# facebookresearch/sylph-few-shot-detection

Measured on AMD Instinct MI355X. Metric: query images/sec, R50-FPN 5-way 5-shot 800x1333 (whole job), higher is better.
Workload: dtype bf16

## Files before the change

### sylph-few-shot-detection_amd/csrc/stem_conv.hip

```cpp
#include "gfx950.h"
#include "kernels.h"

namespace sylph {

namespace {
constexpr int PP = 48;
constexpr int PROWS = 21, PCOLS = 38;
constexpr int PATCH_BYTES = 8192;
constexpr int SCP = 68;
constexpr int NLOAD = (PROWS * PCOLS + 255) / 256;
}

__global__ __launch_bounds__(256, 2) void stem_conv_kernel(const bf16_t* __restrict__ x, const bf16_t* __restrict__ wp,
                                                           const float* __restrict__ scale, const float* __restrict__ shift,
                                                           bf16_t* __restrict__ out, int H, int W, int H2, int W2,
                                                           int tiles_y, int tiles_x, int ntiles) {
  extern __shared__ __attribute__((aligned(16))) char smem[];
  char* patch = smem;
  float* sC = reinterpret_cast<float*>(smem + PATCH_BYTES);
  const int tid = threadIdx.x, lane = tid & 63, wave = tid >> 6, l31 = lane & 31, lh = lane >> 5;

  bf16x8 wb[14][2];
#pragma unroll
  for (int ks = 0; ks < 14; ++ks)
#pragma unroll
    for (int j = 0; j < 2; ++j) wb[ks][j] = *reinterpret_cast<const bf16x8*>(wp + (j * 32 + l31) * 224 + ks * 16 + lh * 8);

  const int m = wave * 32 + l31, py = m >> 4, px = m & 15;
  const int aoff = ((2 * py) * PP + 2 * px + 2 * lh) * 8;

  const int c8 = tid & 7, rr = tid >> 3;
  float sc[8], sh[8];
#pragma unroll
  for (int h = 0; h < 2; ++h) {
    const float4 s4 = reinterpret_cast<const float4*>(scale + c8 * 8)[h], b4 = reinterpret_cast<const float4*>(shift + c8 * 8)[h];
    sc[4 * h] = s4.x; sc[4 * h + 1] = s4.y; sc[4 * h + 2] = s4.z; sc[4 * h + 3] = s4.w;
    sh[4 * h] = b4.x; sh[4 * h + 1] = b4.y; sh[4 * h + 2] = b4.z; sh[4 * h + 3] = b4.w;
  }

  int f_pr[NLOAD], f_pc[NLOAD], f_lds[NLOAD];
  uint32_t f_in = 0;
#pragma unroll
  for (int r = 0; r < NLOAD; ++r) {
    const int idx = tid + 256 * r;
    f_pr[r] = idx / PCOLS; f_pc[r] = idx - f_pr[r] * PCOLS;
    f_lds[r] = (f_pr[r] * PP + f_pc[r]) * 8;
    f_in |= (idx < PROWS * PCOLS ? 1u : 0u) << r;
  }

  auto fetch = [&](int tile_in, uint2 (&v)[NLOAD], uint32_t& okmask) {
    const int tile = tile_in < ntiles ? tile_in : ntiles - 1;
    const int tx = tile % tiles_x, t2 = tile / tiles_x, ty = t2 % tiles_y, b = t2 / tiles_y;
    const int iy0 = ty * 16 - 3, ix0 = tx * 32 - 3;
    okmask = 0;
    const bf16_t* xb = x + (size_t)b * H * W * 4;
#pragma unroll
    for (int r = 0; r < NLOAD; ++r) {
      const int iy = iy0 + f_pr[r], ix = ix0 + f_pc[r];
      const bool ok = ((f_in >> r) & 1u) && (unsigned)iy < (unsigned)H && (unsigned)ix < (unsigned)W;
      const int cy = min(max(iy, 0), H - 1), cx = min(max(ix, 0), W - 1);
      const bf16_t* src = xb + (cy * W + cx) * 4;
      asm volatile("global_load_dwordx2 %0, %1, off" : "=v"(v[r]) : "v"(src) : "memory");
      okmask |= (ok ? 1u : 0u) << r;
    }
  };
  auto park = [&](const uint2 (&v)[NLOAD], uint32_t okmask) {
#pragma unroll
    for (int r = 0; r < NLOAD; ++r) {
      const uint2 t = ((okmask >> r) & 1u) ? v[r] : make_uint2(0u, 0u);
      if ((f_in >> r) & 1u) *reinterpret_cast<uint2*>(patch + f_lds[r]) = t;
    }
  };

#pragma unroll
  for (int ks = 0; ks < 14; ++ks)
#pragma unroll
    for (int j = 0; j < 2; ++j) asm volatile("" : "+v"(wb[ks][j]));
#pragma unroll
  for (int e = 0; e < 8; ++e) { asm volatile("" : "+v"(sc[e])); asm volatile("" : "+v"(sh[e])); }

  const int g = gridDim.x;
  auto do_tile = [&](int tile, uint2 (&q)[NLOAD], uint32_t& qm) {
    wait_vmcnt<4>();
    static_assert(NLOAD == 4, "the vmcnt immediate above is NLOAD");
    park(q, qm);
    lds_barrier();
    fetch(tile + 2 * g, q, qm);

    f32x16 acc[2];
#pragma unroll
    for (int j = 0; j < 2; ++j)
#pragma unroll
      for (int r = 0; r < 16; ++r) acc[j][r] = 0.f;
#pragma unroll
    for (int kh = 0; kh < 7; ++kh)
#pragma unroll
      for (int h = 0; h < 2; ++h) {
        const bf16x8 fa = *reinterpret_cast<const bf16x8*>(patch + aoff + (kh * PP + 4 * h) * 8);
#pragma unroll
        for (int j = 0; j < 2; ++j) acc[j] = __builtin_amdgcn_mfma_f32_32x32x16_bf16(wb[kh * 2 + h][j], fa, acc[j], 0, 0, 0);
      }

    const int tx = tile % tiles_x, t2 = tile / tiles_x, ty = t2 % tiles_y, b = t2 / tiles_y;
    const int oy0 = ty * 8, ox0 = tx * 16;
#pragma unroll
    for (int p = 0; p < 2; ++p) {
      if (p > 0) lds_barrier();
      if ((wave >> 1) == p) {
#pragma unroll
        for (int j = 0; j < 2; ++j)
#pragma unroll
          for (int q4 = 0; q4 < 4; ++q4)
            *reinterpret_cast<float4*>(sC + ((wave & 1) * 32 + l31) * SCP + j * 32 + 8 * q4 + 4 * lh) =
                make_float4(acc[j][4 * q4], acc[j][4 * q4 + 1], acc[j][4 * q4 + 2], acc[j][4 * q4 + 3]);
      }
      lds_barrier();
#pragma unroll
      for (int it = 0; it < 2; ++it) {
        const int rl = rr + 32 * it, mm = p * 64 + rl;
        const int oy = oy0 + (mm >> 4), ox = ox0 + (mm & 15);
        if (oy < H2 && ox < W2) {
          const float4 lo = *reinterpret_cast<const float4*>(sC + rl * SCP + c8 * 8);
          const float4 hi = *reinterpret_cast<const float4*>(sC + rl * SCP + c8 * 8 + 4);
          float v[8] = {lo.x, lo.y, lo.z, lo.w, hi.x, hi.y, hi.z, hi.w};
#pragma unroll
          for (int e = 0; e < 8; ++e) { v[e] = v[e] * sc[e] + sh[e]; v[e] = v[e] > 0.f ? v[e] : 0.f; }
          store8<bf16_t>(out + (((size_t)b * H2 + oy) * W2 + ox) * 64 + c8 * 8, v);
        }
      }
    }
    lds_barrier();
  };

  uint2 qa[NLOAD], qb[NLOAD];
  uint32_t ma, mb;
  int tile = blockIdx.x;
  fetch(tile, qa, ma);
  fetch(tile + g, qb, mb);
  while (tile < ntiles) {
    do_tile(tile, qa, ma);
    tile += g;
    if (tile >= ntiles) break;
    do_tile(tile, qb, mb);
    tile += g;
  }
}

namespace {
constexpr int FR = 17, FC = 15;
constexpr int FPR = 8, FPC = 7;
constexpr int FPROWS = 2 * FR + 5, FPCOLS = 36;
constexpr int FPATCH_BYTES = 15104;
constexpr int FTP = 144;
constexpr int FTILE_BYTES = FR * FC * FTP;
constexpr int FNLOAD = (FPROWS * FPCOLS + 255) / 256;
constexpr int FLDS = FPATCH_BYTES + ((FTILE_BYTES + 127) / 128) * 128 + 128 * 4;
}

struct StemRawArgs { const ImageDesc* imgs; int B; float m0, m1, m2, is0, is1, is2; };

template <bool RAW>
__global__ __launch_bounds__(256, 2) void stem_pool_kernel(const bf16_t* __restrict__ x, const StemRawArgs raw, const bf16_t* __restrict__ wp,
                                                           const float* __restrict__ scale, const float* __restrict__ shift,
                                                           bf16_t* __restrict__ out, char* __restrict__ trash, int H, int W, int H2,
                                                           int W2, int H4, int W4, int tiles_y, int tiles_x, int ntiles) {
  constexpr int NV = RAW ? 3 * FNLOAD : FNLOAD;
  extern __shared__ __attribute__((aligned(16))) char smem[];
  char* patch = smem;
  char* st = smem + FPATCH_BYTES;
  float* ss = reinterpret_cast<float*>(smem + FPATCH_BYTES + ((FTILE_BYTES + 127) / 128) * 128);
  ImageDesc* descs = reinterpret_cast<ImageDesc*>(smem + FLDS);
  const int tid = threadIdx.x, lane = tid & 63, wave = tid >> 6, l31 = lane & 31, lh = lane >> 5;
  if (RAW)
    for (int i = tid; i < raw.B; i += 256) descs[i] = raw.imgs[i];

  bf16x8 wb[14][2];
#pragma unroll
  for (int ks = 0; ks < 14; ++ks)
#pragma unroll
    for (int j = 0; j < 2; ++j) wb[ks][j] = *reinterpret_cast<const bf16x8*>(wp + (j * 32 + l31) * 224 + ks * 16 + lh * 8);
  if (tid < 128) ss[tid] = tid < 64 ? scale[tid] : shift[tid - 64];

  int aoff[2], sy[2], sx[2], toff[2];
#pragma unroll
  for (int p = 0; p < 2; ++p) {
    const int m = min(p * 128 + wave * 32 + l31, FR * FC - 1);
    sy[p] = m / FC;
    sx[p] = m - sy[p] * FC;
    aoff[p] = ((2 * sy[p]) * PP + 2 * sx[p] + 2 * lh) * 8;
    toff[p] = (p * 128 + wave * 32 + l31 < FR * FC) ? m * FTP + 8 * lh : -1;
  }
  int f_pr[FNLOAD], f_pc[FNLOAD], f_lds[FNLOAD];
  uint32_t f_in = 0;
#pragma unroll
  for (int r = 0; r < FNLOAD; ++r) {
    const int idx = tid + 256 * r;
    f_pr[r] = idx / FPCOLS; f_pc[r] = idx - f_pr[r] * FPCOLS;
    f_lds[r] = (f_pr[r] * PP + f_pc[r]) * 8;
    f_in |= (idx < FPROWS * FPCOLS ? 1u : 0u) << r;
  }
  int p_off[2], p_oy[2], p_ox[2];
#pragma unroll
  for (int r = 0; r < 2; ++r) {
    const int idx = tid + 256 * r, pp = idx >> 3;
    p_oy[r] = pp / FPC; p_ox[r] = pp - p_oy[r] * FPC;
    p_off[r] = pp < FPR * FPC ? ((2 * p_oy[r]) * FC + 2 * p_ox[r]) * FTP + (idx & 7) * 16 : -1;
  }
  char* const my_trash = trash + ((size_t)blockIdx.x * 256 + tid) * 16;

  auto tile_origin = [&](int tile, int& b, int& oy0, int& ox0) {
    const int tx = tile % tiles_x, t2 = tile / tiles_x, ty = t2 % tiles_y;
    b = t2 / tiles_y; oy0 = ty * FPR; ox0 = tx * FPC;
  };
  auto fetch = [&](int tile_in, unsigned (&v)[3 * FNLOAD], uint32_t& okmask) {
    int b, oy0, ox0;
    tile_origin(tile_in < ntiles ? tile_in : ntiles - 1, b, oy0, ox0);
    const int iy0 = 4 * oy0 - 5, ix0 = 4 * ox0 - 5;
    okmask = 0;
    if (RAW) {
      const ImageDesc d = descs[b];
      const size_t plane = (size_t)d.h * d.w;
#pragma unroll
      for (int r = 0; r < FNLOAD; ++r) {
        const int iy = iy0 + f_pr[r], ix = ix0 + f_pc[r];
        const bool ok = ((f_in >> r) & 1u) && (unsigned)iy < (unsigned)d.h && (unsigned)ix < (unsigned)d.w;
        const int cy = min(max(iy, 0), d.h - 1), cx = min(max(ix, 0), d.w - 1);
        const float* src = d.ptr + (size_t)cy * d.w + cx;
        asm volatile("global_load_dword %0, %1, off" : "=v"(v[3 * r]) : "v"(src) : "memory");
        asm volatile("global_load_dword %0, %1, off" : "=v"(v[3 * r + 1]) : "v"(src + plane) : "memory");
        asm volatile("global_load_dword %0, %1, off" : "=v"(v[3 * r + 2]) : "v"(src + 2 * plane) : "memory");
        okmask |= (ok ? 1u : 0u) << r;
      }
    } else {
      const bf16_t* xb = x + (size_t)b * H * W * 4;
#pragma unroll
      for (int r = 0; r < FNLOAD; ++r) {
        const int iy = iy0 + f_pr[r], ix = ix0 + f_pc[r];
        const bool ok = ((f_in >> r) & 1u) && (unsigned)iy < (unsigned)H && (unsigned)ix < (unsigned)W;
        const int cy = min(max(iy, 0), H - 1), cx = min(max(ix, 0), W - 1);
        const bf16_t* src = xb + (cy * W + cx) * 4;
        uint2 t;
        asm volatile("global_load_dwordx2 %0, %1, off" : "=v"(t) : "v"(src) : "memory");
        v[2 * r] = t.x; v[2 * r + 1] = t.y;
        okmask |= (ok ? 1u : 0u) << r;
      }
    }
  };
  auto park = [&](const unsigned (&v)[3 * FNLOAD], uint32_t okmask) {
#pragma unroll
    for (int r = 0; r < FNLOAD; ++r) {
      uint2 t = make_uint2(0u, 0u);
      if ((okmask >> r) & 1u) {
        if (RAW) {
          bf16x2 lo2;
          lo2[0] = (bf16_t)((__uint_as_float(v[3 * r]) - raw.m0) * raw.is0);
          lo2[1] = (bf16_t)((__uint_as_float(v[3 * r + 1]) - raw.m1) * raw.is1);
          bf16x2 hi2;
          hi2[0] = (bf16_t)((__uint_as_float(v[3 * r + 2]) - raw.m2) * raw.is2);
          hi2[1] = (bf16_t)0.f;
          t = make_uint2(__builtin_bit_cast(unsigned, lo2), __builtin_bit_cast(unsigned, hi2));
        } else {
          t = make_uint2(v[2 * r], v[2 * r + 1]);
        }
      }
      if ((f_in >> r) & 1u) *reinterpret_cast<uint2*>(patch + f_lds[r]) = t;
    }
  };
#pragma unroll
  for (int ks = 0; ks < 14; ++ks)
#pragma unroll
    for (int j = 0; j < 2; ++j) asm volatile("" : "+v"(wb[ks][j]));
  wait_vmcnt<0>();
  if (RAW) __syncthreads();

  const int g = gridDim.x;
  int nth = 0;
  auto do_tile = [&](int tile, unsigned (&q)[3 * FNLOAD], uint32_t& qm) {
    static_assert(FNLOAD == 6, "the vmcnt immediates below are NV = 6 / 18 (+ 2 stores per finished tile)");
    if (nth == 0) wait_vmcnt<NV>();
    else if (nth == 1) wait_vmcnt<NV + 2>();
    else wait_vmcnt<NV + 4>();
    ++nth;
    park(q, qm);
    lds_barrier();
    fetch(tile + 2 * g, q, qm);
    int b, oy0, ox0;
    tile_origin(tile, b, oy0, ox0);
    const int sy0 = 2 * oy0 - 1, sx0 = 2 * ox0 - 1;
#pragma unroll
    for (int p = 0; p < 2; ++p) {
      f32x16 acc[2];
#pragma unroll
      for (int j = 0; j < 2; ++j)
#pragma unroll
        for (int r = 0; r < 16; ++r) acc[j][r] = 0.f;
#pragma unroll
      for (int kh = 0; kh < 7; ++kh)
#pragma unroll
        for (int h = 0; h < 2; ++h) {
          const bf16x8 fa = *reinterpret_cast<const bf16x8*>(patch + aoff[p] + (kh * PP + 4 * h) * 8);
#pragma unroll
          for (int j = 0; j < 2; ++j) acc[j] = __builtin_amdgcn_mfma_f32_32x32x16_bf16(wb[kh * 2 + h][j], fa, acc[j], 0, 0, 0);
        }
      const bool inimg = (unsigned)(sy0 + sy[p]) < (unsigned)H2 && (unsigned)(sx0 + sx[p]) < (unsigned)W2;
      const unsigned keep = inimg ? 0xffffffffu : 0u;
      if (toff[p] >= 0) {
#pragma unroll
        for (int j = 0; j < 2; ++j)
#pragma unroll
          for (int q4 = 0; q4 < 4; ++q4) {
            const int n0 = 32 * j + 8 * q4 + 4 * lh;
            const f32x4 sv = *reinterpret_cast<const f32x4*>(ss + n0), bv = *reinterpret_cast<const f32x4*>(ss + 64 + n0);
            u32x2 o;
#pragma unroll
            for (int hh = 0; hh < 2; ++hh) {
              bf16x2 v2;
              v2[0] = (bf16_t)(acc[j][4 * q4 + 2 * hh] * sv[2 * hh] + bv[2 * hh]);
              v2[1] = (bf16_t)(acc[j][4 * q4 + 2 * hh + 1] * sv[2 * hh + 1] + bv[2 * hh + 1]);
              const s16x2 z = {0, 0};
              o[hh] = __builtin_bit_cast(unsigned, __builtin_elementwise_max(__builtin_bit_cast(s16x2, v2), z)) & keep;
            }
            *reinterpret_cast<u32x2*>(st + toff[p] + 64 * j + 16 * q4) = o;
          }
      }
    }
    lds_barrier();
#pragma unroll
    for (int r = 0; r < 2; ++r) {
      typedef unsigned short u16x8 __attribute__((ext_vector_type(8)));
      u16x8 mx = {0, 0, 0, 0, 0, 0, 0, 0};
      if (p_off[r] >= 0) {
#pragma unroll
        for (int dy = 0; dy < 3; ++dy)
#pragma unroll
          for (int dx = 0; dx < 3; ++dx)
            mx = __builtin_elementwise_max(mx, *reinterpret_cast<const u16x8*>(st + p_off[r] + (dy * FC + dx) * FTP));
      }
      const int oy = oy0 + p_oy[r], ox = ox0 + p_ox[r];
      const bool okp = p_off[r] >= 0 && oy < H4 && ox < W4;
      char* dst = okp ? reinterpret_cast<char*>(out) + ((((size_t)b * H4 + oy) * W4 + ox) * 64 + (tid & 7) * 8) * 2 : my_trash;
      *reinterpret_cast<u16x8*>(dst) = mx;
    }
    lds_barrier();
  };

  unsigned qa[3 * FNLOAD], qb[3 * FNLOAD];
  uint32_t ma, mb;
  int tile = blockIdx.x;
  fetch(tile, qa, ma);
  fetch(tile + g, qb, mb);
  while (tile < ntiles) {
    do_tile(tile, qa, ma);
    tile += g;
    if (tile >= ntiles) break;
    do_tile(tile, qb, mb);
    tile += g;
  }
}

int launch_stem_pool(const void* x, const void* wp, const float* scale, const float* shift, void* out, void* trash, int B, int H, int W,
                     int H2, int W2, int H4, int W4, hipStream_t s) {
  const int tiles_y = (H4 + FPR - 1) / FPR, tiles_x = (W4 + FPC - 1) / FPC, ntiles = B * tiles_y * tiles_x;
  const int grid = ntiles < 512 ? ntiles : 512;
  hipLaunchKernelGGL(stem_pool_kernel<false>, dim3(grid), dim3(256), FLDS, s, (const bf16_t*)x, StemRawArgs{}, (const bf16_t*)wp, scale, shift,
                     (bf16_t*)out, (char*)trash, H, W, H2, W2, H4, W4, tiles_y, tiles_x, ntiles);
  return (int)hipGetLastError();
}

int launch_stem_pool_raw(const ImageDesc* imgs_dev, const float* mean, const float* stdv, const void* wp, const float* scale,
                         const float* shift, void* out, void* trash, int B, int H, int W, int H2, int W2, int H4, int W4, hipStream_t s) {
  if (B > STEM_RAW_MAX_BATCH) return -1;
  const int tiles_y = (H4 + FPR - 1) / FPR, tiles_x = (W4 + FPC - 1) / FPC, ntiles = B * tiles_y * tiles_x;
  const int grid = ntiles < 512 ? ntiles : 512;
  const StemRawArgs raw{imgs_dev, B, mean[0], mean[1], mean[2], 1.f / stdv[0], 1.f / stdv[1], 1.f / stdv[2]};
  hipLaunchKernelGGL(stem_pool_kernel<true>, dim3(grid), dim3(256), FLDS + (size_t)B * sizeof(ImageDesc), s, (const bf16_t*)nullptr, raw,
                     (const bf16_t*)wp, scale, shift, (bf16_t*)out, (char*)trash, H, W, H2, W2, H4, W4, tiles_y, tiles_x, ntiles);
  return (int)hipGetLastError();
}

int launch_stem_conv(const void* x, const void* wp, const float* scale, const float* shift, void* out, int B, int H, int W, int H2,
                     int W2, hipStream_t s) {
  const int tiles_y = (H2 + 7) / 8, tiles_x = (W2 + 15) / 16, ntiles = B * tiles_y * tiles_x;
  const int grid = ntiles < 512 ? ntiles : 512;
  const size_t lds = PATCH_BYTES + (size_t)64 * SCP * 4;
  hipLaunchKernelGGL(stem_conv_kernel, dim3(grid), dim3(256), lds, s, (const bf16_t*)x, (const bf16_t*)wp, scale, shift, (bf16_t*)out,
                     H, W, H2, W2, tiles_y, tiles_x, ntiles);
  return (int)hipGetLastError();
}

}
```

Before: 2334.

## Software-pipeline LDS reads and interleave next-tile fetches with MFMA in stem pool kernel

Reworks the fused stem conv+maxpool kernel. The double-buffered two-tiles-ahead prefetch becomes a single buffer whose global loads for the next tile are issued one chunk at a time between MFMA steps. LDS reads for the A fragments, the scale/shift values and the pooling taps are issued ahead through inline-asm ds_read_b128 with explicit lgkmcnt waits, so LDS latency overlaps compute. The patch layout gets padding (FPP 46 plus extra bytes every two rows) and the pooling lanes are remapped, presumably to reduce bank conflicts. In exchange the prefetch distance drops to one tile, which may expose more global-load latency, and the hand-written waitcnt counts are fragile.

After: 2331. Within noise of the previous version (-0.1%).

```diff
diff --git a/sylph-few-shot-detection_amd/csrc/stem_conv.hip b/sylph-few-shot-detection_amd/csrc/stem_conv.hip
--- a/sylph-few-shot-detection_amd/csrc/stem_conv.hip
+++ b/sylph-few-shot-detection_amd/csrc/stem_conv.hip
@@ -1,3 +1,5 @@
+#include <utility>
+
 #include "gfx950.h"
 #include "kernels.h"
 
@@ -155,6 +157,43 @@
 constexpr int FTILE_BYTES = FR * FC * FTP;
 constexpr int FNLOAD = (FPROWS * FPCOLS + 255) / 256;
 constexpr int FLDS = FPATCH_BYTES + ((FTILE_BYTES + 127) / 128) * 128 + 128 * 4;
+constexpr int FPP = 46;
+__device__ __forceinline__ constexpr int fpatch_off(int pr, int pc) { return (pr * FPP + pc) * 8 + (pr >> 1) * 16; }
+static_assert(fpatch_off(2 * FR + 4, 36) <= 15104, "the patch fits FPATCH_BYTES");
+constexpr int FD = 5;
+constexpr int SD = 4;
+
+__device__ __forceinline__ unsigned lds_addr(const void* p) { return (unsigned)(size_t)(__attribute__((address_space(3))) const char*)p; }
+template <int OFF, class T> __device__ __forceinline__ void lds_read16(T& d, unsigned ad) {
+  static_assert(sizeof(T) == 16 && OFF >= 0 && OFF < 65536, "ds_read_b128, 16-bit offset");
+  asm volatile("ds_read_b128 %0, %1 offset:%2" : "=v"(d) : "v"(ad), "n"(OFF));
+}
+template <int OFF> __device__ __forceinline__ void lds_write8(unsigned ad, const u32x2& v) {
+  static_assert(OFF >= 0 && OFF < 65536, "16-bit offset");
+  asm volatile("ds_write_b64 %0, %1 offset:%2" ::"v"(ad), "v"(v), "n"(OFF) : "memory");
+}
+template <int N, class T> __device__ __forceinline__ void lds_wait(T& a) { asm volatile("s_waitcnt lgkmcnt(%1)" : "+v"(a) : "n"(N)); }
+template <int N, class T> __device__ __forceinline__ void lds_wait(T& a, T& b) {
+  asm volatile("s_waitcnt lgkmcnt(%2)" : "+v"(a), "+v"(b) : "n"(N));
+}
+template <class F, int... I> __device__ __forceinline__ void static_for_impl(F&& f, std::integer_sequence<int, I...>) {
+  (f(std::integral_constant<int, I>{}), ...);
+}
+template <int N, class F> __device__ __forceinline__ void static_for(F&& f) { static_for_impl(f, std::make_integer_sequence<int, N>{}); }
+template <int N, bool RAW> __device__ __forceinline__ void patch_landed(unsigned (&q)[3 * FNLOAD]) {
+  if constexpr (RAW)
+    asm volatile("s_waitcnt vmcnt(%18)"
+                 : "+v"(q[0]), "+v"(q[1]), "+v"(q[2]), "+v"(q[3]), "+v"(q[4]), "+v"(q[5]), "+v"(q[6]), "+v"(q[7]), "+v"(q[8]), "+v"(q[9]),
+                   "+v"(q[10]), "+v"(q[11]), "+v"(q[12]), "+v"(q[13]), "+v"(q[14]), "+v"(q[15]), "+v"(q[16]), "+v"(q[17])
+                 : "n"(N)
+                 : "memory");
+  else
+    asm volatile("s_waitcnt vmcnt(%12)"
+                 : "+v"(q[0]), "+v"(q[1]), "+v"(q[2]), "+v"(q[3]), "+v"(q[4]), "+v"(q[5]), "+v"(q[6]), "+v"(q[7]), "+v"(q[8]), "+v"(q[9]),
+                   "+v"(q[10]), "+v"(q[11])
+                 : "n"(N)
+                 : "memory");
+}
 }
 
 struct StemRawArgs { const ImageDesc* imgs; int B; float m0, m1, m2, is0, is1, is2; };
@@ -164,7 +203,6 @@
                                                            const float* __restrict__ scale, const float* __restrict__ shift,
                                                            bf16_t* __restrict__ out, char* __restrict__ trash, int H, int W, int H2,
                                                            int W2, int H4, int W4, int tiles_y, int tiles_x, int ntiles) {
-  constexpr int NV = RAW ? 3 * FNLOAD : FNLOAD;
   extern __shared__ __attribute__((aligned(16))) char smem[];
   char* patch = smem;
   char* st = smem + FPATCH_BYTES;
@@ -181,70 +219,72 @@
     for (int j = 0; j < 2; ++j) wb[ks][j] = *reinterpret_cast<const bf16x8*>(wp + (j * 32 + l31) * 224 + ks * 16 + lh * 8);
   if (tid < 128) ss[tid] = tid < 64 ? scale[tid] : shift[tid - 64];
 
-  int aoff[2], sy[2], sx[2], toff[2];
+  int sy[2], sx[2];
+  unsigned a_lds[2], t_lds[2];
 #pragma unroll
   for (int p = 0; p < 2; ++p) {
     const int m = min(p * 128 + wave * 32 + l31, FR * FC - 1);
     sy[p] = m / FC;
     sx[p] = m - sy[p] * FC;
-    aoff[p] = ((2 * sy[p]) * PP + 2 * sx[p] + 2 * lh) * 8;
-    toff[p] = (p * 128 + wave * 32 + l31 < FR * FC) ? m * FTP + 8 * lh : -1;
-  }
-  int f_pr[FNLOAD], f_pc[FNLOAD], f_lds[FNLOAD];
+    a_lds[p] = lds_addr(patch) + fpatch_off(2 * sy[p], 2 * sx[p] + 2 * lh);
+    t_lds[p] = lds_addr(st) + m * FTP + 8 * lh;
+  }
+  const unsigned ss_lds = lds_addr(ss) + 16 * lh;
+  int f_rc[FNLOAD];
   uint32_t f_in = 0;
 #pragma unroll
   for (int r = 0; r < FNLOAD; ++r) {
-    const int idx = tid + 256 * r;
-    f_pr[r] = idx / FPCOLS; f_pc[r] = idx - f_pr[r] * FPCOLS;
-    f_lds[r] = (f_pr[r] * PP + f_pc[r]) * 8;
+    const int idx = tid + 256 * r, pr = idx / FPCOLS;
+    f_rc[r] = pr << 8 | (idx - pr * FPCOLS);
     f_in |= (idx < FPROWS * FPCOLS ? 1u : 0u) << r;
   }
   int p_off[2], p_oy[2], p_ox[2];
+  const int p_qd = (lane & 31) >> 2, p_chunk = ((0x96 >> p_qd) & 1) * 4 + (lane & 3);
 #pragma unroll
   for (int r = 0; r < 2; ++r) {
-    const int idx = tid + 256 * r, pp = idx >> 3;
+    const int pp = 8 * (wave + 4 * r) + 2 * (p_qd >> 1) + lh;
     p_oy[r] = pp / FPC; p_ox[r] = pp - p_oy[r] * FPC;
-    p_off[r] = pp < FPR * FPC ? ((2 * p_oy[r]) * FC + 2 * p_ox[r]) * FTP + (idx & 7) * 16 : -1;
-  }
+    p_off[r] = pp < FPR * FPC ? ((2 * p_oy[r]) * FC + 2 * p_ox[r]) * FTP + p_chunk * 16 : -1;
+  }
+  const unsigned p_lds[2] = {lds_addr(st) + max(p_off[0], 0), lds_addr(st) + max(p_off[1], 0)};
   char* const my_trash = trash + ((size_t)blockIdx.x * 256 + tid) * 16;
 
   auto tile_origin = [&](int tile, int& b, int& oy0, int& ox0) {
     const int tx = tile % tiles_x, t2 = tile / tiles_x, ty = t2 % tiles_y;
     b = t2 / tiles_y; oy0 = ty * FPR; ox0 = tx * FPC;
   };
-  auto fetch = [&](int tile_in, unsigned (&v)[3 * FNLOAD], uint32_t& okmask) {
+  struct Fetch { const float* ptr; const bf16_t* xb; size_t plane; int h, w, iy0, ix0; };
+  auto fetch_begin = [&](int tile_in) {
     int b, oy0, ox0;
     tile_origin(tile_in < ntiles ? tile_in : ntiles - 1, b, oy0, ox0);
-    const int iy0 = 4 * oy0 - 5, ix0 = 4 * ox0 - 5;
-    okmask = 0;
+    Fetch f;
+    f.iy0 = 4 * oy0 - 5; f.ix0 = 4 * ox0 - 5;
     if (RAW) {
       const ImageDesc d = descs[b];
-      const size_t plane = (size_t)d.h * d.w;
-#pragma unroll
-      for (int r = 0; r < FNLOAD; ++r) {
-        const int iy = iy0 + f_pr[r], ix = ix0 + f_pc[r];
-        const bool ok = ((f_in >> r) & 1u) && (unsigned)iy < (unsigned)d.h && (unsigned)ix < (unsigned)d.w;
-        const int cy = min(max(iy, 0), d.h - 1), cx = min(max(ix, 0), d.w - 1);
-        const float* src = d.ptr + (size_t)cy * d.w + cx;
-        asm volatile("global_load_dword %0, %1, off" : "=v"(v[3 * r]) : "v"(src) : "memory");
-        asm volatile("global_load_dword %0, %1, off" : "=v"(v[3 * r + 1]) : "v"(src + plane) : "memory");
-        asm volatile("global_load_dword %0, %1, off" : "=v"(v[3 * r + 2]) : "v"(src + 2 * plane) : "memory");
-        okmask |= (ok ? 1u : 0u) << r;
-      }
+      f.ptr = d.ptr; f.xb = nullptr; f.h = d.h; f.w = d.w; f.plane = (size_t)d.h * d.w;
     } else {
-      const bf16_t* xb = x + (size_t)b * H * W * 4;
-#pragma unroll
-      for (int r = 0; r < FNLOAD; ++r) {
-        const int iy = iy0 + f_pr[r], ix = ix0 + f_pc[r];
-        const bool ok = ((f_in >> r) & 1u) && (unsigned)iy < (unsigned)H && (unsigned)ix < (unsigned)W;
-        const int cy = min(max(iy, 0), H - 1), cx = min(max(ix, 0), W - 1);
-        const bf16_t* src = xb + (cy * W + cx) * 4;
-        uint2 t;
-        asm volatile("global_load_dwordx2 %0, %1, off" : "=v"(t) : "v"(src) : "memory");
-        v[2 * r] = t.x; v[2 * r + 1] = t.y;
-        okmask |= (ok ? 1u : 0u) << r;
-      }
-    }
+      f.ptr = nullptr; f.xb = x + (size_t)b * H * W * 4; f.h = H; f.w = W; f.plane = 0;
+    }
+    return f;
+  };
+  auto fetch_chunk = [&](const Fetch& f, int r, unsigned (&v)[3 * FNLOAD], uint32_t& okmask) {
+    int rc = f_rc[r];
+    asm volatile("" : "+v"(rc));
+    const int iy = f.iy0 + (rc >> 8), ix = f.ix0 + (rc & 255);
+    const bool ok = ((f_in >> r) & 1u) && (unsigned)iy < (unsigned)f.h && (unsigned)ix < (unsigned)f.w;
+    const int cy = min(max(iy, 0), f.h - 1), cx = min(max(ix, 0), f.w - 1);
+    if (RAW) {
+      const float* src = f.ptr + (size_t)cy * f.w + cx;
+      asm volatile("global_load_dword %0, %1, off" : "=v"(v[3 * r]) : "v"(src) : "memory");
+      asm volatile("global_load_dword %0, %1, off" : "=v"(v[3 * r + 1]) : "v"(src + f.plane) : "memory");
+      asm volatile("global_load_dword %0, %1, off" : "=v"(v[3 * r + 2]) : "v"(src + 2 * f.plane) : "memory");
+    } else {
+      const bf16_t* src = f.xb + (cy * f.w + cx) * 4;
+      uint2 t;
+      asm volatile("global_load_dwordx2 %0, %1, off" : "=v"(t) : "v"(src) : "memory");
+      v[2 * r] = t.x; v[2 * r + 1] = t.y;
+    }
+    okmask |= (ok ? 1u : 0u) << r;
   };
   auto park = [&](const unsigned (&v)[3 * FNLOAD], uint32_t okmask) {
 #pragma unroll
@@ -263,7 +303,9 @@
           t = make_uint2(v[2 * r], v[2 * r + 1]);
         }
       }
-      if ((f_in >> r) & 1u) *reinterpret_cast<uint2*>(patch + f_lds[r]) = t;
+      int rc = f_rc[r];
+      asm volatile("" : "+v"(rc));
+      if ((f_in >> r) & 1u) *reinterpret_cast<uint2*>(patch + fpatch_off(rc >> 8, rc & 255)) = t;
     }
   };
 #pragma unroll
@@ -274,87 +316,108 @@
   if (RAW) __syncthreads();
 
   const int g = gridDim.x;
-  int nth = 0;
-  auto do_tile = [&](int tile, unsigned (&q)[3 * FNLOAD], uint32_t& qm) {
-    static_assert(FNLOAD == 6, "the vmcnt immediates below are NV = 6 / 18 (+ 2 stores per finished tile)");
-    if (nth == 0) wait_vmcnt<NV>();
-    else if (nth == 1) wait_vmcnt<NV + 2>();
-    else wait_vmcnt<NV + 4>();
-    ++nth;
+  unsigned q[3 * FNLOAD];
+  uint32_t qm = 0;
+  auto do_tile = [&](int tile) {
     park(q, qm);
     lds_barrier();
-    fetch(tile + 2 * g, q, qm);
+    const Fetch nf = fetch_begin(tile + g);
+    qm = 0;
     int b, oy0, ox0;
     tile_origin(tile, b, oy0, ox0);
     const int sy0 = 2 * oy0 - 1, sx0 = 2 * ox0 - 1;
 #pragma unroll
     for (int p = 0; p < 2; ++p) {
+      bf16x8 af[FD];
+      f32x4 sv[SD], bv[SD];
+      static_for<FD - 1>([&](auto kc) {
+        constexpr int k = decltype(kc)::value;
+        lds_read16<fpatch_off(k >> 1, 4 * (k & 1))>(af[k], a_lds[p]);
+      });
       f32x16 acc[2];
 #pragma unroll
       for (int j = 0; j < 2; ++j)
 #pragma unroll
         for (int r = 0; r < 16; ++r) acc[j][r] = 0.f;
-#pragma unroll
-      for (int kh = 0; kh < 7; ++kh)
-#pragma unroll
-        for (int h = 0; h < 2; ++h) {
-          const bf16x8 fa = *reinterpret_cast<const bf16x8*>(patch + aoff[p] + (kh * PP + 4 * h) * 8);
-#pragma unroll
-          for (int j = 0; j < 2; ++j) acc[j] = __builtin_amdgcn_mfma_f32_32x32x16_bf16(wb[kh * 2 + h][j], fa, acc[j], 0, 0, 0);
-        }
+      static_for<14>([&](auto kc) {
+        constexpr int k = decltype(kc)::value, kn = k + FD - 1;
+        if constexpr (kn < 14) lds_read16<fpatch_off(kn >> 1, 4 * (kn & 1))>(af[kn % FD], a_lds[p]);
+        lds_wait<(kn < 14 ? FD - 1 : 13 - k)>(af[k % FD]);
+        if constexpr (k == 13) {
+          static_for<SD - 1>([&](auto ic) {
+            constexpr int i = decltype(ic)::value;
+            lds_read16<32 * i>(sv[i], ss_lds);
+            lds_read16<256 + 32 * i>(bv[i], ss_lds);
+          });
+        }
+#pragma unroll
+        for (int j = 0; j < 2; ++j) acc[j] = __builtin_amdgcn_mfma_f32_32x32x16_bf16(wb[k][j], af[k % FD], acc[j], 0, 0, 0);
+        if constexpr ((k & 1) == 0 && k / 2 < FNLOAD) {
+          if (p == 0) fetch_chunk(nf, k / 2, q, qm);
+        }
+      });
       const bool inimg = (unsigned)(sy0 + sy[p]) < (unsigned)H2 && (unsigned)(sx0 + sx[p]) < (unsigned)W2;
       const unsigned keep = inimg ? 0xffffffffu : 0u;
-      if (toff[p] >= 0) {
-#pragma unroll
-        for (int j = 0; j < 2; ++j)
-#pragma unroll
-          for (int q4 = 0; q4 < 4; ++q4) {
-            const int n0 = 32 * j + 8 * q4 + 4 * lh;
-            const f32x4 sv = *reinterpret_cast<const f32x4*>(ss + n0), bv = *reinterpret_cast<const f32x4*>(ss + 64 + n0);
-            u32x2 o;
-#pragma unroll
-            for (int hh = 0; hh < 2; ++hh) {
-              bf16x2 v2;
-              v2[0] = (bf16_t)(acc[j][4 * q4 + 2 * hh] * sv[2 * hh] + bv[2 * hh]);
-              v2[1] = (bf16_t)(acc[j][4 * q4 + 2 * hh + 1] * sv[2 * hh + 1] + bv[2 * hh + 1]);
-              const s16x2 z = {0, 0};
-              o[hh] = __builtin_bit_cast(unsigned, __builtin_elementwise_max(__builtin_bit_cast(s16x2, v2), z)) & keep;
-            }
-            *reinterpret_cast<u32x2*>(st + toff[p] + 64 * j + 16 * q4) = o;
-          }
-      }
+      static_for<8>([&](auto ic) {
+        constexpr int i = decltype(ic)::value, in = i + SD - 1, j = i >> 2, q4 = i & 3;
+        if constexpr (in < 8) {
+          lds_read16<32 * in>(sv[in % SD], ss_lds);
+          lds_read16<256 + 32 * in>(bv[in % SD], ss_lds);
+        }
+        lds_wait<2 * (in < 8 ? SD - 1 : 7 - i) + (i < SD - 1 ? i : SD - 1)>(sv[i % SD], bv[i % SD]);
+        u32x2 o;
+#pragma unroll
+        for (int hh = 0; hh < 2; ++hh) {
+          bf16x2 v2;
+          v2[0] = (bf16_t)(acc[j][4 * q4 + 2 * hh] * sv[i % SD][2 * hh] + bv[i % SD][2 * hh]);
+          v2[1] = (bf16_t)(acc[j][4 * q4 + 2 * hh + 1] * sv[i % SD][2 * hh + 1] + bv[i % SD][2 * hh + 1]);
+          const s16x2 z = {0, 0};
+          o[hh] = __builtin_bit_cast(unsigned, __builtin_elementwise_max(__builtin_bit_cast(s16x2, v2), z)) & keep;
+        }
+        lds_write8<16 * i>(t_lds[p], o);
+      });
     }
     lds_barrier();
-#pragma unroll
-    for (int r = 0; r < 2; ++r) {
-      typedef unsigned short u16x8 __attribute__((ext_vector_type(8)));
-      u16x8 mx = {0, 0, 0, 0, 0, 0, 0, 0};
-      if (p_off[r] >= 0) {
-#pragma unroll
-        for (int dy = 0; dy < 3; ++dy)
-#pragma unroll
-          for (int dx = 0; dx < 3; ++dx)
-            mx = __builtin_elementwise_max(mx, *reinterpret_cast<const u16x8*>(st + p_off[r] + (dy * FC + dx) * FTP));
-      }
+    typedef unsigned short u16x8 __attribute__((ext_vector_type(8)));
+    u16x8 tap[9], mx[2] = {{0, 0, 0, 0, 0, 0, 0, 0}, {0, 0, 0, 0, 0, 0, 0, 0}};
+    static_for<9>([&](auto tc) {
+      constexpr int t = decltype(tc)::value;
+      lds_read16<((t / 3) * FC + t % 3) * FTP>(tap[t], p_lds[0]);
+    });
+    static_for<9>([&](auto tc) {
+      constexpr int t = decltype(tc)::value;
+      lds_wait<8>(tap[t]);
+      mx[0] = __builtin_elementwise_max(mx[0], tap[t]);
+      lds_read16<((t / 3) * FC + t % 3) * FTP>(tap[t], p_lds[1]);
+    });
+    auto store_pooled = [&](int r) {
       const int oy = oy0 + p_oy[r], ox = ox0 + p_ox[r];
       const bool okp = p_off[r] >= 0 && oy < H4 && ox < W4;
-      char* dst = okp ? reinterpret_cast<char*>(out) + ((((size_t)b * H4 + oy) * W4 + ox) * 64 + (tid & 7) * 8) * 2 : my_trash;
-      *reinterpret_cast<u16x8*>(dst) = mx;
-    }
-    lds_barrier();
-  };
-
-  unsigned qa[3 * FNLOAD], qb[3 * FNLOAD];
-  uint32_t ma, mb;
+      char* dst = okp ? reinterpret_cast<char*>(out) + ((((size_t)b * H4 + oy) * W4 + ox) * 64 + p_chunk * 8) * 2 : my_trash;
+      *reinterpret_cast<u16x8*>(dst) = mx[r];
+    };
+    store_pooled(0);
+    static_for<9>([&](auto tc) {
+      constexpr int t = decltype(tc)::value;
+      lds_wait<8 - t>(tap[t]);
+      mx[1] = __builtin_elementwise_max(mx[1], tap[t]);
+    });
+    store_pooled(1);
+  };
+
+  static_assert(FNLOAD == 6, "patch_landed() names 3 * FNLOAD (RAW) or 2 * FNLOAD registers");
   int tile = blockIdx.x;
-  fetch(tile, qa, ma);
-  fetch(tile + g, qb, mb);
-  while (tile < ntiles) {
-    do_tile(tile, qa, ma);
+  {
+    const Fetch f0 = fetch_begin(tile);
+#pragma unroll
+    for (int r = 0; r < FNLOAD; ++r) fetch_chunk(f0, r, q, qm);
+  }
+  patch_landed<0, RAW>(q);
+  while (true) {
+    do_tile(tile);
     tile += g;
     if (tile >= ntiles) break;
-    do_tile(tile, qb, mb);
-    tile += g;
+    patch_landed<2, RAW>(q);
   }
 }
 
```
